# pierre-borie/Benlsip.jl

Hardware: AMD Instinct MI355X
Metric: PCG subproblems/sec + achieved HBM GB/s, dense m=65536 n=4096 fp64 (higher is better)
Workload: dtype f64

## Files before the change

benlsip.jl_amd/csrc/bh_api.hip:

```cpp
#include "../../include/benlsip_hip.h"
#include "bh_cauchy_plan.h"
#include "bh_free_image_plan.h"
#include "bh_gram_ingest_plan.h"
#include "bh_kernels.hip.h"
#include "bh_launch_ahead.h"
#include "bh_pcg_plan.h"

#include <dlfcn.h>
#include <fcntl.h>
#include <rccl/rccl.h>
#include <sched.h>
#include <sys/mman.h>
#include <unistd.h>

#include <algorithm>
#include <atomic>
#include <chrono>
#include <cmath>
#include <cstdio>
#include <cstdlib>
#include <cstring>
#include <array>
#include <initializer_list>
#include <string>
#include <thread>
#include <tuple>
#include <vector>

using namespace bh;

static uint64_t g_kernel_launches = 0;
static uint64_t g_mask_epoch = 0;
#undef hipLaunchKernelGGL
#define hipLaunchKernelGGL(kernelName, ...) do { ++g_kernel_launches; hipLaunchKernelGGLInternal((kernelName), __VA_ARGS__); } while (0)

namespace {

struct CgWorkspace {
    int64_t n_pad = 0;
    double *w = nullptr, *r = nullptr, *v = nullptr, *p = nullptr, *Hp = nullptr, *g = nullptr, *wl = nullptr, *wu = nullptr;
    double *x = nullptr, *s = nullptr, *xlow = nullptr, *xupp = nullptr;
    double* hw = nullptr;
    double *p2 = nullptr, *gpart = nullptr, *rvpart = nullptr;
    double *r2 = nullptr, *hpx = nullptr, *hpx_tail = nullptr;
    double* slab = nullptr;
    double* scalars = nullptr;
    CgState* d_state = nullptr;
    volatile unsigned long long* h_mirror = nullptr;
    unsigned long long* d_mirror = nullptr;
    unsigned tag = 0;
    unsigned long long* d_reroute = nullptr;
    unsigned long long reroute_seq = 0;
    double* d_trace = nullptr;
    int64_t trace_cap = 0;
};

struct PeerShm {
    std::atomic<int> arrive;
    std::atomic<int> generation;
    int failed;
    hipIpcMemHandle_t handle[kMaxPeers];
};
struct PeerComm {
    bool active = false;
    bool broken = false;
    void* inbox = nullptr;
    size_t inbox_bytes = 0;
    void* peer_base[kMaxPeers] = {};
    volatile unsigned long long* h_err = nullptr;
    PeerShm* shm = nullptr;
    PeerArgs args{};
};
constexpr int64_t kPeerCap = 1 << 16;
constexpr int kPeerBlkCap = (int)(kPeerCap / (2 * kPeerBlockChunks));
constexpr size_t kPeerSlotBytes = (size_t)2 * kMaxPeers * kPeerCap * sizeof(double);
constexpr size_t kPeerFlagBytes = (size_t)2 * kMaxPeers * kPeerBlkCap * sizeof(unsigned long long);
constexpr size_t kPeerScalBytes = kPeerFlagBytes;

struct AsyncUpload {
    std::thread worker;
    int32_t rc = BH_OK;
    std::string detail;
    hipStream_t s_copy = nullptr, s_xpose = nullptr;
    double* staging[2] = {nullptr, nullptr};
    hipEvent_t copied[2] = {nullptr, nullptr}, freed[2] = {nullptr, nullptr};
// ... 9 lines not shown
};

struct Ctx {
    bool init = false;
    int device = -1;
    int flags = 0;
    int n_cu = 0;
    hipStream_t own_stream = nullptr;
    hipStream_t stream = nullptr;
    std::string detail;
    int64_t opt_blocks_per_cu = 0;
    int64_t opt_batch = 0;
    int64_t opt_chol_downdate = 0;
    int64_t opt_cauchy_image = 1;
    int64_t opt_cauchy_image_max_ma = 64;
    int64_t opt_cauchy_image_refresh = 0;
    int64_t opt_cauchy_fused = 1;
    int64_t opt_cauchy_gram_eq = 0;
    int64_t opt_cauchy_gram = 0;
    int64_t opt_linv_refine = 1;
    int64_t opt_cauchy_gemm = 1;
    int64_t opt_gram_cg_fused = 0;
    int64_t opt_gram_mfma = 1;
    int64_t opt_ls_from_cg = 1;
    int64_t opt_step_from_cg = 0;
    struct { const void* H = nullptr; const double* w = nullptr; const double* gm = nullptr; } hw_note;
    struct { const void* H = nullptr; const double* s = nullptr; const double* g = nullptr; const double* gm = nullptr; } gm_note;
    int64_t opt_fold_init = 1;
    int64_t opt_final_sync = 0;
    int64_t opt_host_copy_kernels = 1;
    int64_t opt_cg_fused = 1;
    int64_t opt_proj_form = 1;
    int64_t opt_upload_chunk_mb = 64;
    int64_t opt_free_image = 1;
    int64_t opt_gram_ingest = 0;
    int64_t opt_ev_stride = 8;
    void* rccl_lib = nullptr;
    ncclComm_t comm = nullptr;
    int rank = 0, nranks = 1;
    ncclResult_t (*p_ncclGetUniqueId)(ncclUniqueId*) = nullptr;
    ncclResult_t (*p_ncclCommInitRank)(ncclComm_t*, int, ncclUniqueId, int) = nullptr;
    ncclResult_t (*p_ncclCommDestroy)(ncclComm_t) = nullptr;
    ncclResult_t (*p_ncclAllReduce)(const void*, void*, size_t, ncclDataType_t, ncclRedOp_t, ncclComm_t, hipStream_t) = nullptr;
    const char* (*p_ncclGetErrorString)(ncclResult_t) = nullptr;
    PeerComm peer;
    int comm_path = 0;
    CgWorkspace cg;
    double* scratch_dev = nullptr;
    struct PooledImage { double* ptr; int64_t doubles; };
    std::vector<PooledImage> image_pool;
    int64_t opt_image_pool = 2;
    int64_t image_pool_hits = 0;
    AsyncUpload* upload_cache = nullptr;
    int64_t h2d_bytes = 0, d2h_bytes = 0, h2d_calls = 0, d2h_calls = 0;
    volatile unsigned long long* mbox_h = nullptr;
    unsigned long long* mbox_d = nullptr;
    unsigned long long mbox_seq = 0;
    double* rbuf = nullptr;
    int64_t rbuf_cap = 0;
    int live_hess = 0;
    bool reform_vlds_attr_set = false;
    bool vlds_attr_set = false;
    bool cgp_vlds_attr_set = false;
    bool trsm_lds_granted = false;
    size_t trsv_lds_granted = 0;
};
// ... 273 lines not shown

namespace {

int32_t ensure_cg_workspace(int64_t n_pad, int64_t trace_cap) {
    CgWorkspace& c = g_ctx.cg;
    if (c.n_pad < n_pad) {
        double** vecs[] = {&c.w, &c.r, &c.v, &c.p, &c.Hp, &c.s, &c.x, &c.xlow, &c.xupp, &c.g, &c.wl, &c.wu, &c.hw, &c.p2, &c.gpart, &c.rvpart,
                           &c.r2, &c.hpx, &c.hpx_tail};
        constexpr int NV = 19;
        dev_free(c.slab);
        c.slab = nullptr;
        g_ctx.hw_note = {};
        BH_TRY(dev_alloc(&c.slab, NV * n_pad + 8));
        BH_HIP(hipMemsetAsync(c.slab, 0, (size_t)(NV * n_pad + 8) * sizeof(double), g_ctx.stream));
        for (int i = 0; i < NV; ++i) *vecs[i] = c.slab + (int64_t)i * n_pad;
        c.scalars = c.slab + NV * n_pad;
        c.n_pad = n_pad;
    }
    if (!c.d_state) {
        BH_TRY(dev_alloc(&c.d_state, 1));
        BH_HIP(hipMemsetAsync(c.d_state, 0, sizeof(CgState), g_ctx.stream));
        void* hp = nullptr;
        BH_HIP(hipHostMalloc(&hp, 64, hipHostMallocMapped | hipHostMallocCoherent));
        memset(hp, 0, 64);
        c.h_mirror = reinterpret_cast<volatile unsigned long long*>(hp);
        void* dp = nullptr;
        BH_HIP(hipHostGetDevicePointer(&dp, hp, 0));
        c.d_mirror = reinterpret_cast<unsigned long long*>(dp);
    }
    if (!c.d_reroute) {
        BH_TRY(dev_alloc(&c.d_reroute, 1));
        BH_HIP(hipMemsetAsync(c.d_reroute, 0, sizeof(unsigned long long), g_ctx.stream));
    }
    if (trace_cap > c.trace_cap) {
        dev_free(c.d_trace);
        c.d_trace = nullptr;
        BH_TRY(dev_alloc(&c.d_trace, 4 * trace_cap));
        c.trace_cap = trace_cap;
    }
    return BH_OK;
}

int32_t check_peer_error();
int32_t hess_ready(bh_hess* H);

int32_t wait_mirror(CgWorkspace& c, unsigned tag, int target, MirrorWord* out, int iter_target = 0) {
    const auto t0 = std::chrono::steady_clock::now();
    unsigned long long spins = 0;
    auto reached = [&](unsigned long long w, MirrorWord* m) {
        if (((w >> 48) & 0xffffu) != (tag & 0xffffu)) return false;
        m->status = (int)((w >> 44) & 0xf);
        m->done = (int)((w >> 40) & 0xf);
        m->iter = (int)((w >> 20) & 0xfffff);
        m->n_hmul = (int)(w & 0xfffff);
        return m->done != 0 || m->n_hmul >= target || (iter_target > 0 && m->iter >= iter_target);
    };
    while (true) {
        if (reached(*c.h_mirror, out)) return BH_OK;
        __builtin_ia32_pause();
        if ((++spins & 0xffff) == 0) {
            if (g_ctx.peer.active && *g_ctx.peer.h_err != 0ull) return check_peer_error();
            hipError_t q = hipStreamQuery(g_ctx.stream);
            if (q != hipSuccess && q != hipErrorNotReady) return fail(BH_ERR_HIP, std::string("CG loop: ") + hipGetErrorString(q));
            if (q == hipSuccess) {
                MirrorWord m2{};
                if (!reached(*c.h_mirror, &m2)) return fail(BH_ERR_HIP, "internal: stream drained but the loop state did not reach the launch target");
// ... 756 lines not shown
        default: return "unknown error code";
    }
}

const char* bh_last_error_detail(void) { return g_ctx.detail.c_str(); }

int32_t bh_init(int32_t device, int32_t flags) {
    if (g_ctx.init) {
        if (device != g_ctx.device)
            return fail(BH_ERR_INVALID_ARG, "bh_init: already initialised on another device (bh_shutdown first)");
        g_ctx.flags = flags;
        return BH_OK;
    }
    int count = 0;
    hipError_t e = hipGetDeviceCount(&count);
    if (e != hipSuccess || count <= 0) return fail(BH_ERR_NO_DEVICE, "hipGetDeviceCount found no device");
    if (device < 0 || device >= count) return fail(BH_ERR_INVALID_ARG, "device ordinal out of range");
    BH_HIP(hipSetDevice(device));
    hipDeviceProp_t prop;
    BH_HIP(hipGetDeviceProperties(&prop, device));
    g_ctx.n_cu = prop.multiProcessorCount;
    g_ctx.device = device;
    g_ctx.flags = flags;
    BH_HIP(hipStreamCreateWithFlags(&g_ctx.own_stream, hipStreamNonBlocking));
    g_ctx.stream = g_ctx.own_stream;
    BH_TRY(dev_alloc(&g_ctx.scratch_dev, 1024));
    BH_TRY(mbox_ensure());
    if (const char* s = getenv("BH_HOST_COPY_KERNELS")) g_ctx.opt_host_copy_kernels = atoll(s) ? 1 : 0;
    if (const char* s = getenv("BH_BLOCKS_PER_CU")) g_ctx.opt_blocks_per_cu = std::min<int64_t>(std::max<int64_t>(0, atoll(s)), kMaxBlocksPerCu);
    if (const char* s = getenv("BH_PCG_BATCH")) g_ctx.opt_batch = std::max<int64_t>(0, atoll(s));
    if (const char* s = getenv("BH_PROJ_FORM")) g_ctx.opt_proj_form = atoll(s) ? 1 : 0;
    if (const char* s = getenv("BH_CG_FUSED")) g_ctx.opt_cg_fused = std::min<int64_t>(std::max<int64_t>(0, atoll(s)), 2);
    if (const char* s = getenv("BH_FINAL_SYNC")) g_ctx.opt_final_sync = atoll(s) ? 1 : 0;
    if (const char* s = getenv("BH_FREE_IMAGE")) g_ctx.opt_free_image = std::min<int64_t>(std::max<int64_t>(0, atoll(s)), 2);
    g_ctx.init = true;
    return BH_OK;
}

static void peer_release(bool with_barrier);

int32_t bh_shutdown(void) {
    if (!g_ctx.init) return BH_OK;
    (void)hipStreamSynchronize(g_ctx.stream);
    if (g_ctx.comm && g_ctx.p_ncclCommDestroy) { g_ctx.p_ncclCommDestroy(g_ctx.comm); g_ctx.comm = nullptr; }
    if (g_ctx.peer.active) peer_release(true);
    g_ctx.comm_path = 0;
    CgWorkspace& c = g_ctx.cg;
    dev_free(c.slab); dev_free(c.d_state); dev_free(c.d_trace); dev_free(c.d_reroute);
    if (c.h_mirror) (void)hipHostFree(const_cast<unsigned long long*>(c.h_mirror));
    c = CgWorkspace();
    dev_free(g_ctx.scratch_dev); g_ctx.scratch_dev = nullptr;
    dev_free(g_ctx.rbuf); g_ctx.rbuf = nullptr; g_ctx.rbuf_cap = 0;
    if (g_ctx.mbox_h) { (void)hipHostFree(const_cast<unsigned long long*>(g_ctx.mbox_h)); g_ctx.mbox_h = nullptr; g_ctx.mbox_d = nullptr; }
    async_upload_destroy(g_ctx.upload_cache); g_ctx.upload_cache = nullptr;
    for (auto& im : g_ctx.image_pool) dev_free(im.ptr);
    g_ctx.image_pool.clear();
    if (g_ctx.own_stream) (void)hipStreamDestroy(g_ctx.own_stream);
    g_ctx.own_stream = nullptr; g_ctx.stream = nullptr;
    if (g_pin.base) { (void)hipHostFree(g_pin.base); g_pin = PinArena(); }
    g_ctx.vlds_attr_set = false; g_ctx.cgp_vlds_attr_set = false; g_ctx.reform_vlds_attr_set = false; g_ctx.trsm_lds_granted = false; g_ctx.trsv_lds_granted = 0;
    g_ctx.init = false; g_ctx.rank = 0; g_ctx.nranks = 1;
    return BH_OK;
}

int32_t bh_set_stream(void* hip_stream) {
    BH_REQUIRE_INIT();
    BH_TRY(sync_flush());
    g_ctx.stream = hip_stream ? reinterpret_cast<hipStream_t>(hip_stream) : g_ctx.own_stream;
    return BH_OK;
}

int32_t bh_synchronize(void) {
    BH_REQUIRE_INIT();
    BH_TRY(sync_flush());
    return BH_OK;
}

int32_t bh_device_info(char* name_out, int64_t name_cap, int32_t* n_cu, char* arch_out, int64_t arch_cap) {
    BH_REQUIRE_INIT();
    hipDeviceProp_t prop;
    BH_HIP(hipGetDeviceProperties(&prop, g_ctx.device));
    if (name_out && name_cap > 0) { strncpy(name_out, prop.name, (size_t)name_cap - 1); name_out[name_cap - 1] = 0; }
    if (arch_out && arch_cap > 0) { strncpy(arch_out, prop.gcnArchName, (size_t)arch_cap - 1); arch_out[arch_cap - 1] = 0; }
    if (n_cu) *n_cu = prop.multiProcessorCount;
    return BH_OK;
}

int32_t bh_set_option(const char* key, int64_t value) {
    if (!key) return fail(BH_ERR_INVALID_ARG, "NULL key");
    if (!strcmp(key, "blocks_per_cu")) {
        if (value < 0 || value > kMaxBlocksPerCu) return fail(BH_ERR_INVALID_ARG, "blocks_per_cu must be 0 (default) .. 8");
        g_ctx.opt_blocks_per_cu = value;
        return BH_OK;
    }
    if (!strcmp(key, "pcg_batch")) { g_ctx.opt_batch = std::max<int64_t>(0, value); return BH_OK; }
    if (!strcmp(key, "proj_form")) { g_ctx.opt_proj_form = value ? 1 : 0; return BH_OK; }
    if (!strcmp(key, "fold_init")) { g_ctx.opt_fold_init = value ? 1 : 0; return BH_OK; }
    if (!strcmp(key, "cg_fused")) {
        if (value < 0 || value > 2) return fail(BH_ERR_INVALID_ARG, "cg_fused is 0, 1 (box constraints) or 2 (also linear equalities)");
        g_ctx.opt_cg_fused = value;
        return BH_OK;
    }
    if (!strcmp(key, "final_sync")) { g_ctx.opt_final_sync = value ? 1 : 0; return BH_OK; }
    if (!strcmp(key, "host_copy_kernels")) { g_ctx.opt_host_copy_kernels = value ? 1 : 0; return BH_OK; }
    if (!strcmp(key, "ls_from_cg")) { g_ctx.opt_ls_from_cg = value ? 1 : 0; return BH_OK; }
    if (!strcmp(key, "step_from_cg")) { g_ctx.opt_step_from_cg = value ? 1 : 0; return BH_OK; }
    if (!strcmp(key, "gram_mfma")) { g_ctx.opt_gram_mfma = value; return BH_OK; }
    if (!strcmp(key, "chol_downdate")) { g_ctx.opt_chol_downdate = value ? 1 : 0; return BH_OK; }
    if (!strcmp(key, "cauchy_image")) { g_ctx.opt_cauchy_image = value ? 1 : 0; return BH_OK; }
    if (!strcmp(key, "cauchy_gram")) { g_ctx.opt_cauchy_gram = value ? 1 : 0; return BH_OK; }
    if (!strcmp(key, "cauchy_gram_eq")) {
        if (value != 0 && value != 1) return fail(BH_ERR_INVALID_ARG, "cauchy_gram_eq is 0 or 1");
        g_ctx.opt_cauchy_gram_eq = value;
        return BH_OK;
    }
    if (!strcmp(key, "gram_cg_fused")) {
        if (value != 0) BH_REQUIRE_INIT();
        if (value != 0 && value != 1) return fail(BH_ERR_INVALID_ARG, "gram_cg_fused is 0 or 1");
        g_ctx.opt_gram_cg_fused = value;
        return BH_OK;
    }
    if (!strcmp(key, "cauchy_image_refresh")) {
        if (value < 0) return fail(BH_ERR_INVALID_ARG, "cauchy_image_refresh is 0 (never) or the number of passes between two re-formations");
        g_ctx.opt_cauchy_image_refresh = value;
        return BH_OK;
    }
    if (!strcmp(key, "cauchy_fused")) { g_ctx.opt_cauchy_fused = value ? 1 : 0; return BH_OK; }
    if (!strcmp(key, "linv_refine")) { g_ctx.opt_linv_refine = value ? 1 : 0; return BH_OK; }
    if (!strcmp(key, "cauchy_gemm")) { g_ctx.opt_cauchy_gemm = value ? 1 : 0; return BH_OK; }
    if (!strcmp(key, "cauchy_image_max_ma")) { g_ctx.opt_cauchy_image_max_ma = std::min<int64_t>(std::max<int64_t>(0, value), 64); return BH_OK; }
    if (!strcmp(key, "image_pool")) {
        if (value < 0 || value > 8) return fail(BH_ERR_INVALID_ARG, "image_pool must be 0..8");
        g_ctx.opt_image_pool = value;
        while ((int64_t)g_ctx.image_pool.size() > value) { dev_free(g_ctx.image_pool.back().ptr); g_ctx.image_pool.pop_back(); }
        return BH_OK;
// ... 986 lines not shown
        cold = 1;
    }
    p.sched.first = launch_ahead_first(H->last_n_hmul, cold);
    return p;
}

static void pcg_use_free_image(PcgRun& r) {
    bh_hess* H = r.H; CgWorkspace& c = r.c;
    const FreeImageBook& b = H->fi;
    r.fi_use = true;
    r.og = c.x; r.owl = c.xlow; r.owu = c.xupp; r.ow = c.s;
    r.ofix = nullptr;
    r.on = (int)b.nfree; r.onch = (int)(round_up(b.nfree, 16) / 2);
    r.old = b.ldf;
    pcg_fused_geometry(r.plan, H, r.onch, r.on);
    H->call_bytes = free_image_bytes(H);
    c.reroute_seq += 1;
}

static int32_t pcg_fused_stream(PcgRun& r, int j) {
    bh_hess* H = r.H; CgWorkspace& c = r.c; const PcgPlan& p = r.plan;
    RowStreamArgs ra = rs_args(H, p.nrows, nullptr);
    ra.partials = H->partials;
    if (p.gram) { ra.J = H->G; ra.d_rows = p.nrows; ra.mu = 1.0; ra.partials = nullptr; ra.t_out = c.Hp; }
    if (r.fi_use) { ra.J = H->Jf; ra.ld = r.old; ra.nchunks = r.onch; }
    if (p.sel.fuse_gen) { ra.v = c.p; ra.negate = 0; }
    else { ra.v = r.og; ra.negate = 1; ra.negmask = r.ofix; }
    CgFuse& f = ra.cf;
    f.st = c.d_state; f.j = j; f.n = r.on; f.max_iter = p.max_iter; f.init_done = p.sel.gen_linv ? 2 : p.sel.fuse_gen ? 1 : 0; f.vv_off = p.vv_off;
    f.vvec = c.v; f.p_old = p.pbuf[(j - 1) & 1]; f.p_new = p.pbuf[j & 1];
    f.rvpart = p.rvbuf[(j - 1) & 1]; f.nrv = p.nrv;
    f.w = r.ow; f.wl = r.owl; f.wu = r.owu;
    if (r.fi_use) { f.reroute = c.d_reroute; f.reroute_seq = c.reroute_seq; }
    f.sqpart = H->sq_partials; f.gpart = H->sq_partials + H->g_cap;
    f.kappa2 = r.a.kappa2; f.atol_f2b = r.a.atol_f2b;
    f.trace = r.a.trace; f.trace_cap = r.a.trace_cap; f.mirror = r.a.mirror; f.tag = r.a.tag;
    int slot = -1;
    const bool expect_stop = j == r.expect_stop_at || j > p.max_iter || (r.expect_stop_at == 0 && j > 1);
    BH_TRY(profile_begin(H, j - 1, &slot));
    if (p.gram) launch_gram_cg(p.cfg, ra, p.grid, r.s, expect_stop);
    else launch_row_stream_cgp(p.cfg, ra, p.grid, r.s, expect_stop);
    if (slot >= 0) BH_HIP(hipEventRecord(H->ev[2 * slot + 1], r.s));
    return BH_OK;
}

static int32_t pcg_fused_update(PcgRun& r, int j) {
    bh_hess* H = r.H; bh_proj* P = r.P; CgWorkspace& c = r.c; const PcgPlan& p = r.plan; hipStream_t s = r.s;
    const int nblk = p.nblk, grid = p.grid;
    CgUpdArgs u{};
    u.st = c.d_state; u.j = j; u.partials = H->partials; u.ld = r.old; u.nchunks = r.onch; u.G = grid; u.Gs = grid; u.Gq = grid;
    u.sqpart = H->sq_partials; u.gpart = H->sq_partials + H->g_cap; u.rvpart_in = p.rvbuf[(j - 1) & 1]; u.rvpart_out = p.rvbuf[j & 1]; u.nrv = p.nrv;
    u.p = p.pbuf[j & 1]; u.w = r.ow; u.hw = r.hw; u.r = c.r; u.g = r.og; u.v = c.v; u.fixrank = r.ofix;
    if (r.fi_use) { u.map = H->fi_map; u.w_full = r.wp; u.reroute = c.d_reroute; u.reroute_seq = c.reroute_seq; }
    u.n = r.on; u.atol_neg = r.a.atol_neg; u.trace = r.a.trace; u.trace_cap = r.a.trace_cap; u.mirror = r.a.mirror; u.tag = r.a.tag;
    if (p.gram) { u.partials = c.Hp; u.Gs = 1; }
    if (!p.sel.fuse_gen) {
        if (p.sel.peer_fused) hipLaunchKernelGGL((cg_reduce_update_kernel<false, true>), dim3(nblk), dim3(256), 0, s, u, g_ctx.peer.args);
        else hipLaunchKernelGGL((cg_reduce_update_kernel<false, false>), dim3(nblk), dim3(256), 0, s, u, PeerArgs{});
        return BH_OK;
    }
    if (p.sel.rccl_gen) {
        const int n_pad = r.a.n_pad;
        hipLaunchKernelGGL(reduce_partials_sq_kernel, dim3(nblk), dim3(256), 0, s, (const double*)H->partials, H->ld, H->nchunks, grid,
                           c.hpx, (const double*)H->sq_partials, n_pad, (const CgState*)c.d_state, j);
        BH_HIP(hipGetLastError());
        BH_TRY(allreduce_inplace(c.hpx, (int64_t)n_pad + 2, H));
        u.partials = c.hpx; u.Gs = 1; u.sqpart = c.hpx + n_pad; u.Gq = 1;
    }
    u.A = P->Ad; u.ldA = P->ldA; u.mA = (int)P->mA; u.tpart = P->tpart; u.init_in_memory = p.sel.gen_linv ? 0 : 1;
    if (p.sel.peer_fused) hipLaunchKernelGGL((cg_reduce_update_kernel<true, true>), dim3(nblk), dim3(256), 0, s, u, g_ctx.peer.args);
    else hipLaunchKernelGGL((cg_reduce_update_kernel<true, false>), dim3(nblk), dim3(256), 0, s, u, PeerArgs{});
    ProjArgs pa = proj_args(P, c.d_state, true);
    pa.tpart = P->tpart; pa.tpart_nblk = nblk; pa.rvpart = p.rvbuf[j & 1]; pa.fused_j = j;
    if (p.sel.gen_linv) {
        pa.W = P->W; pa.nch_pad = H->nchunks; pa.Mgram = p.sel.linv_refine ? P->M : nullptr;
        hipLaunchKernelGGL((proj_apply_linv_kernel<false>), dim3((unsigned)p.nrv), dim3(256), 0, s, pa, (const double*)c.r, c.v);
        return BH_OK;
    }
    hipLaunchKernelGGL(trsv_small_kernel, dim3(1), dim3(256), 0, s, pa);
    hipLaunchKernelGGL((proj_left_mul_tr_kernel<true, 4>), dim3((p.nch_v + 63) / 64), dim3(256), 0, s, pa, (const double*)c.r, c.v);
    return BH_OK;
}

static int32_t pcg_fused_first(PcgRun& r) {
    bh_hess* H = r.H; bh_proj* P = r.P; CgWorkspace& c = r.c; const PcgPlan& p = r.plan; hipStream_t s = r.s;
    if (r.fi_use) {
        FreeGatherArgs ga{};
        ga.g = r.a.g; ga.wl = r.a.wl; ga.wu = r.a.wu; ga.fixrank = P->fixrank; ga.map = H->fi_map;
        ga.gc = c.x; ga.wlc = c.xlow; ga.wuc = c.xupp; ga.wc = c.s; ga.w = r.wp;
        ga.n = r.a.n; ga.n_pad = r.a.n_pad; ga.nfree = r.on;
        ga.reroute = c.d_reroute; ga.seq = c.reroute_seq; ga.mirror = r.a.mirror; ga.tag = r.a.tag;
        hipLaunchKernelGGL(free_image_gather_kernel, dim3((unsigned)((r.a.n_pad + 255) / 256)), dim3(256), 0, s, ga);
    }
    if (p.sel.gen_linv) {
        if (!P->linv_valid) {
            hipLaunchKernelGGL(tri_inv_small_kernel, dim3(1), dim3(256), 0, s, (const double*)P->Lr, (int)P->mA, P->W);
            P->linv_valid = true;
        }
        ProjArgs pa = proj_args(P, nullptr, true);
        hipLaunchKernelGGL(proj_left_mul_kernel, dim3((unsigned)P->mA), dim3(256), 0, s, pa, r.a.g);
        pa.tpart = P->tw; pa.tpart_nblk = 1; pa.rvpart = p.rvbuf[0]; pa.vvpart = p.rvbuf[0] + p.vv_off; pa.p_out = c.p;
        pa.W = P->W; pa.nch_pad = H->nchunks; pa.Mgram = p.sel.linv_refine ? P->M : nullptr; pa.fused_j = 0;
        hipLaunchKernelGGL((proj_apply_linv_kernel<true>), dim3((unsigned)p.nrv), dim3(256), 0, s, pa, r.a.g, c.v);
    } else if (p.sel.fuse_gen) {
        hipLaunchKernelGGL((cg_init_kernel<false>), dim3(1), dim3(CG_T), 0, s, r.a);
        BH_TRY(launch_project(P, c.r, c.v, c.d_state));
        hipLaunchKernelGGL(cg_init_finish_kernel, dim3(1), dim3(CG_T), 0, s, r.a);
    }
    return pcg_fused_stream(r, 1);
}

static int32_t pcg_fused_unit(PcgRun& r, int index) {
    BH_TRY(pcg_fused_update(r, index + 1));
    BH_TRY(pcg_fused_stream(r, index + 2));
    BH_HIP(hipGetLastError());
    return BH_OK;
}

static int32_t pcg_rccl_box_stream(PcgRun& r, int j) {
    bh_hess* H = r.H; CgWorkspace& c = r.c; const PcgPlan& p = r.plan; const CgArgs& a = r.a;
    RowStreamArgs ra = rs_args(H, p.nrows, nullptr);
    ra.partials = H->partials;
    ra.v = a.g; ra.negate = 1; ra.negmask = a.fixrank;
    CgFuse& f = ra.cf;
    f.st = c.d_state; f.j = j; f.n = a.n; f.max_iter = p.max_iter; f.init_done = 0;
    f.p_old = p.pbuf[(j - 1) & 1]; f.p_new = p.pbuf[j & 1];
// ... 1165 lines not shown
```

benlsip.jl_amd/csrc/bh_cg.hip.h:

```cpp
#pragma once
#include <hip/hip_runtime.h>
#include <stdint.h>
#include "bh_reduce.hip.h"

namespace bh {

constexpr int CG_T = 1024;

struct CgArgs {
    CgState* st;
    double* w; double* r; double* v; double* p;
    const double* Hp;
    const double* g;
    const double* wl; const double* wu;
    const int* fixrank;
    int n;
    int n_pad;
    int w_in_ws;
    int max_iter;
    double kappa2, atol_neg, atol_f2b;
    double* trace; int trace_cap;
    double* hw;
    unsigned long long* mirror;
    unsigned tag;
};

__device__ __forceinline__ double f2b_term(double p, double w, double wl, double wu, double atol) {
    double g = __longlong_as_double(0x7ff0000000000000ll);
    if (p <= -atol) g = __ddiv_rn(__dsub_rn(wl, w), p);
    else if (p >= atol) g = __ddiv_rn(__dsub_rn(wu, w), p);
    return g;
}

__device__ __forceinline__ int cg_final_status(const CgState* st) {
    if (st->approx_solved) return 0;
    if (st->outside_region) return 1;
    if (st->neg_curvature) return 2;
    if (st->iter == st->max_iter) return 3;
    return 4;
}

__device__ __forceinline__ void publish_state(const CgArgs& a, const CgState* st) {
    if (a.mirror == nullptr) return;
    const unsigned long long wv = ((unsigned long long)(a.tag & 0xffffu) << 48) | ((unsigned long long)(st->status & 0xf) << 44) |
                                  ((unsigned long long)(st->done & 0xf) << 40) | ((unsigned long long)(st->iter & 0xfffff) << 20) |
                                  (unsigned long long)(st->n_hmul & 0xfffff);
    if (st->done) {
        const unsigned long long tw = ((unsigned long long)(st->margin_kind & 0xf) << 48) | ((unsigned long long)(st->tie_flags & 0xff) << 40) |
                                      ((unsigned long long)(st->tie_first & 0xfffff) << 20) | (unsigned long long)(st->margin_at & 0xfffff);
        __hip_atomic_store(a.mirror + 1, tw, __ATOMIC_RELAXED, __HIP_MEMORY_SCOPE_SYSTEM);
        __hip_atomic_store(a.mirror + 2, (unsigned long long)__double_as_longlong(st->min_margin), __ATOMIC_RELAXED, __HIP_MEMORY_SCOPE_SYSTEM);
    }
    __hip_atomic_store(a.mirror, wv, __ATOMIC_RELAXED, __HIP_MEMORY_SCOPE_SYSTEM);
}

__device__ __forceinline__ void publish_word(unsigned long long* mirror, unsigned tag, int status, int done, int iter, int n_hmul,
                                             const TieRegs& tr) {
    if (mirror == nullptr) return;
    const unsigned long long wv = ((unsigned long long)(tag & 0xffffu) << 48) | ((unsigned long long)(status & 0xf) << 44) |
                                  ((unsigned long long)(done & 0xf) << 40) | ((unsigned long long)(iter & 0xfffff) << 20) |
                                  (unsigned long long)(n_hmul & 0xfffff);
    if (done) {
        const unsigned long long tw = ((unsigned long long)(tr.margin_kind & 0xf) << 48) | ((unsigned long long)(tr.tie_flags & 0xff) << 40) |
                                      ((unsigned long long)(tr.tie_first & 0xfffff) << 20) | (unsigned long long)(tr.margin_at & 0xfffff);
        __hip_atomic_store(mirror + 1, tw, __ATOMIC_RELAXED, __HIP_MEMORY_SCOPE_SYSTEM);
        __hip_atomic_store(mirror + 2, (unsigned long long)__double_as_longlong(tr.min_margin), __ATOMIC_RELAXED, __HIP_MEMORY_SCOPE_SYSTEM);
    }
    __hip_atomic_store(mirror, wv, __ATOMIC_RELAXED, __HIP_MEMORY_SCOPE_SYSTEM);
}
__device__ __forceinline__ int cg_status_of(int approx_solved, int outside_region, int neg_curvature, int iter, int max_iter) {
    if (approx_solved) return 0;
    if (outside_region) return 1;
    if (neg_curvature) return 2;
// ... 471 lines not shown
```

benlsip.jl_amd/csrc/bh_cgfuse.hip.h:

```cpp
#pragma once
#include <hip/hip_runtime.h>
#include <stdint.h>
#include "bh_reduce.hip.h"
#include "bh_cg.hip.h"
#include "bh_comm.hip.h"

namespace bh {

struct CgUpdArgs {
    CgState* st;
    int j;
    const double* partials; int64_t ld; int nchunks; int G;
    int Gs, Gq;
    const double* sqpart;
    const double* gpart;
    const double* rvpart_in;
    double* rvpart_out;
    int nrv;
    const double* p;
    double* w; double* hw;
    double* r; const double* g;
    double* v;
    const int* fixrank;
    int n;
    double atol_neg;
    double* trace; int trace_cap;
    unsigned long long* mirror; unsigned tag;
    const double* A; int64_t ldA; int mA;
    double* tpart;
    int init_in_memory;
    const int* map; double* w_full;
    const unsigned long long* reroute; unsigned long long reroute_seq;
};

template <bool GEN, bool PEER>
__global__ __launch_bounds__(256) void cg_reduce_update_kernel(CgUpdArgs a, PeerArgs pa) {
    CgState* st = a.st;
    if (st->stop_at != 0 && a.j > st->stop_at) return;
    if (a.reroute != nullptr && *a.reroute == a.reroute_seq) return;
    __shared__ double2 sm[16][17];
    __shared__ double rvs[16];
    __shared__ double2 rsm[16];
    const int tid = threadIdx.x, cl = tid & 15, rl = tid >> 4;
    const int c = blockIdx.x * 16 + cl;
    const bool valid = c < a.nchunks;
    const int64_t ld2 = a.ld >> 1;
    const double QNAN = __longlong_as_double(0x7ff8000000000000ll);

    const bool upd = (rl == 0) && valid;
    const bool from_g = (a.j == 1 && !a.init_in_memory);
    double2 pk = make_double2(0.0, 0.0), wk = pk, hwk = pk, rk = pk;
    int2 fr = make_int2(-1, -1);
    if (upd) {
        pk = reinterpret_cast<const double2*>(a.p)[c];
        if (from_g) {
            rk = reinterpret_cast<const double2*>(a.g)[c];
        } else {
            rk = reinterpret_cast<const double2*>(a.r)[c];
            wk = reinterpret_cast<const double2*>(a.w)[c];
            if (a.hw != nullptr) hwk = reinterpret_cast<const double2*>(a.hw)[c];
        }
    }
    TieRegs tr;
    tr.load(st);
    const int max_iter = st->max_iter;
    const double rtv_state = st->rtv;
    LaneBatch<8> b_sq, b_gp, b_rv;
    b_sq.issue(a.sqpart, a.Gq);
    b_gp.issue(a.gpart, a.G);
    b_rv.issue(a.rvpart_in, a.nrv);
    const double2* P2 = reinterpret_cast<const double2*>(a.partials);
    const int cc = min(c, a.nchunks - 1);
    SlabBatch sb;
    sb.issue(P2, ld2, cc, rl, a.Gs);
    double2 arow[4];
    if (GEN) {
        const double2* A2 = reinterpret_cast<const double2*>(a.A);
        const int64_t ldA2 = a.ldA >> 1;
#pragma unroll
        for (int k = 0; k < 4; ++k) arow[k] = A2[(int64_t)min(rl + 16 * k, a.mA - 1) * ldA2 + cc];
    }
    int2 mp = make_int2(-1, -1);
    if (!GEN && upd && a.map != nullptr) mp = reinterpret_cast<const int2*>(a.map)[c];
    if (upd && a.fixrank != nullptr) fr = reinterpret_cast<const int2*>(a.fixrank)[c];

    const double2 acc = sb.fold(P2, ld2, cc, rl, a.Gs);
    sm[rl][cl] = acc;

    double pHp = wave_sum(b_sq.fold_sum(a.sqpart, a.Gq));
    if (PEER) {
        __shared__ int s_timeout;
        __shared__ double2 xs[kMaxPeers][16];
        __shared__ double ps[kMaxPeers];
        if (tid == 0) s_timeout = 0;
        __syncthreads();
        if (rl == 0) {
            double2 t = sm[0][cl];
#pragma unroll
            for (int q = 1; q < 16; ++q) { t.x += sm[q][cl].x; t.y += sm[q][cl].y; }
// ... 112 lines not shown
    } else {
        __syncthreads();
        if (cont) {
            const double2 rm = rsm[cl];
#pragma unroll
            for (int k = 0; k < 4; ++k) {
                const int i = rl + 16 * k;
                if (i < a.mA) {
                    double prod = valid ? fma(arow[k].y, rm.y, arow[k].x * rm.x) : 0.0;
                    prod = row16_sum(prod);
                    if (cl == 0) a.tpart[(int64_t)blockIdx.x * a.mA + i] = prod;
                }
            }
        }
    }

    if (blockIdx.x == 0 && tid == 0) {
        st->pHp = pHp; st->gamma = gamma; st->alpha = alpha; st->n_hmul = a.j; st->rtv = rtv;
        st->neg_curvature = neg; st->outside_region = outside; st->need_proj = 0; st->iter = a.j;
        tr.note_step_a(pHp, a.atol_neg, alpha, gamma, a.j);
        tr.store(st);
        if (a.trace != nullptr && a.j <= a.trace_cap) {
            double* row = a.trace + 4 * (int64_t)(a.j - 1);
            row[0] = pHp; row[1] = alpha; row[2] = (neg && !add_w) ? QNAN : gamma; row[3] = rtv;
        }
        int status = 4;
        if (!cont) {
            status = cg_status_of(0, outside, neg, a.j, max_iter);
            st->approx_solved = 0; st->done = 1; st->stop_at = a.j;
            st->status = status;
        }
        publish_word(a.mirror, a.tag, status, cont ? 0 : 1, a.j, a.j, tr);
    }
}

}
```

benlsip.jl_amd/csrc/bh_freeimg.hip.h:

```cpp
#pragma once
#include <hip/hip_runtime.h>
#include <stdint.h>
#include "bh_reduce.hip.h"

namespace bh {

__global__ __launch_bounds__(256) void free_image_build_kernel(const double* __restrict__ J, int64_t ld, int64_t nrows,
                                                               const int* __restrict__ map, double* __restrict__ Jf, int64_t ldf) {
    const int nch = (int)(ldf >> 1);
    for (int64_t row = blockIdx.x; row < nrows; row += gridDim.x) {
        const double* __restrict__ src = J + row * ld;
        double2* __restrict__ dst = reinterpret_cast<double2*>(Jf + row * ldf);
        for (int c = threadIdx.x; c < nch; c += 256) {
            const int2 m = reinterpret_cast<const int2*>(map)[c];
            double2 x = make_double2(0.0, 0.0);
            if (m.x >= 0 && m.y == m.x + 1 && (m.x & 1) == 0) {
                const dvec2 t = __builtin_nontemporal_load(reinterpret_cast<const dvec2*>(src + m.x));
                x = make_double2(t.x, t.y);
            } else {
                if (m.x >= 0) x.x = __builtin_nontemporal_load(src + m.x);
                if (m.y >= 0) x.y = __builtin_nontemporal_load(src + m.y);
            }
            dst[c] = x;
        }
    }
}

__global__ __launch_bounds__(256) void free_image_move_kernel(double* __restrict__ Jf, int64_t ldf, int64_t nrows, int nfree_new, int k,
                                                              const int* __restrict__ dst_of_tail, int* __restrict__ map) {
    const int64_t total = nrows * (int64_t)k;
    for (int64_t idx = (int64_t)blockIdx.x * 256 + threadIdx.x; idx < total; idx += (int64_t)gridDim.x * 256) {
        const int64_t row = idx / k;
        const int t = (int)(idx - row * k);
        const int dst = dst_of_tail[t];
        double* __restrict__ rp = Jf + row * ldf;
        const double x = rp[nfree_new + t];
        if (dst >= 0) rp[dst] = x;
        rp[nfree_new + t] = 0.0;
    }
    if (blockIdx.x == 0) {
        for (int t = threadIdx.x; t < k; t += 256) {
            const int dst = dst_of_tail[t];
            const int var = map[nfree_new + t];
            if (dst >= 0) map[dst] = var;
            map[nfree_new + t] = -1;
        }
    }
}

constexpr int kCgReroute = 15;
struct FreeGatherArgs {
    const double* g; const double* wl; const double* wu;
    const int* fixrank;
    const int* map;
    double* gc; double* wlc; double* wuc;
    double* wc;
    double* w;
    int n, n_pad, nfree;
    unsigned long long* reroute; unsigned long long seq;
    unsigned long long* mirror; unsigned tag;
};

__global__ __launch_bounds__(256) void free_image_gather_kernel(FreeGatherArgs a) {
    const int i = blockIdx.x * 256 + threadIdx.x;
    if (i < a.n_pad) {
        const int m = (i < a.nfree) ? a.map[i] : -1;
        a.gc[i] = (m >= 0) ? a.g[m] : 0.0;
        a.wlc[i] = (m >= 0) ? a.wl[m] : 0.0;
        a.wuc[i] = (m >= 0) ? a.wu[m] : 0.0;
        a.wc[i] = 0.0;
    }
    if (i < a.n && a.fixrank[i] >= 0) {
        a.w[i] = 0.0;
        const double gi = a.g[i];
        if (!(fabs(gi) <= 1.7976931348623157e308)) {
            *a.reroute = a.seq;
            if (a.mirror != nullptr) {
                const unsigned long long wv = ((unsigned long long)(a.tag & 0xffffu) << 48) | ((unsigned long long)kCgReroute << 44) | (1ull << 40);
                __hip_atomic_store(a.mirror, wv, __ATOMIC_RELAXED, __HIP_MEMORY_SCOPE_SYSTEM);
            }
        }
    }
}

}
```

benlsip.jl_amd/csrc/bh_matvec.hip.h:

```cpp
#pragma once
#include <hip/hip_runtime.h>
#include <stdint.h>
#include "bh_reduce.hip.h"
#include "bh_cg.hip.h"

namespace bh {

enum { MODE_JV = 0, MODE_JTV = 1, MODE_FUSED = 2 };

struct CgFuse {
    CgState* st;
    int j;
    int init_done;
    int vv_off;
    int n, max_iter;
    const double* vvec;
    const double* p_old;
    double* p_new;
    const double* rvpart;
    int nrv;
    const double* w;
    const double* wl; const double* wu;
    double* sqpart;
    double* gpart;
    double kappa2, atol_f2b;
    double* trace; int trace_cap;
    unsigned long long* mirror; unsigned tag;
    const double* gpart_in;
    const double* Hp;
    int sq_index;
    const double* r_old;
    double* r_new;
    double* w_rw;
    double* hw;
    const double* g;
    const int* fixrank;
    double atol_neg;
    const unsigned long long* reroute; unsigned long long reroute_seq;
};

struct RowStreamArgs {
    const double* J;
    int64_t ld;
    int64_t nrows;
    int64_t d_rows;
    int nchunks;
    const double* v;
    const double* u;
    double* t_out;
    double* partials;
    double* sq_partials;
    double mu;
    const CgState* state;
    int accumulate;
    int weighted_u;
    int negate;
    const int* negmask;
    CgFuse cf;
};

template <int T, int CPT, int R, int MODE, int NT = 1, int PF = 1, int VL = 0, int CGP = 0>
__global__ __launch_bounds__(T) void row_stream_kernel(RowStreamArgs a) {
    static_assert(NT == 1 && PF == 1, "plain loads (NT = 0) and the single register buffer (PF = 0) lost their A/Bs and were removed");
    if (!CGP && a.state != nullptr && a.state->done) return;
    if (CGP && a.cf.j > 1 && a.cf.st->stop_at != 0 && a.cf.j > a.cf.st->stop_at + (CGP == 3 ? 1 : 0)) return;
    if ((CGP == 1 || CGP == 2) && a.cf.reroute != nullptr && *a.cf.reroute == a.cf.reroute_seq) return;
    constexpr int NW = T / 64;
    __shared__ double red[2][R][NW];
    __shared__ double pro[2][NW];
    extern __shared__ __attribute__((aligned(16))) double2 v_lds[];

    const int tid = threadIdx.x, lane = tid & 63, wave = tid >> 6;
    const int64_t ld2 = a.ld >> 1;
    const double2* __restrict__ J2 = reinterpret_cast<const double2*>(a.J);
    const int64_t ngroups = (a.nrows + R - 1) / R;
    const int64_t G = gridDim.x;

    bool act[CPT];
    double2 vv[CPT], zz[CPT];
#pragma unroll
    for (int k = 0; k < CPT; ++k) act[k] = (tid + k * T) < a.nchunks;

    double2 A[R][CPT], B[R][CPT];
    double sq_acc = 0.0;
    int buf = 0;

    auto load_group = [&](double2 (&dst)[R][CPT], int64_t grp) {
#pragma unroll
        for (int r = 0; r < R; ++r) {
            const int64_t row = grp * R + r;
            const bool rv = row < a.nrows;
            const double2* rp = J2 + (rv ? row : 0) * ld2;
#pragma unroll
            for (int k = 0; k < CPT; ++k) {
                dst[r][k] = make_double2(0.0, 0.0);
                if (rv && act[k]) {
                    const dvec2 t = __builtin_nontemporal_load(reinterpret_cast<const dvec2*>(rp + tid + k * T));
                    dst[r][k] = make_double2(t.x, t.y);
                }
// ... 40 lines not shown
            if (tid < R && row < a.nrows) a.t_out[row] = a.accumulate ? a.t_out[row] + mine : mine;
        }
#pragma unroll
        for (int r = 0; r < R; ++r) {
            const int64_t row = grp * R + r;
            const bool rv = row < a.nrows;
            if (MODE == MODE_JV) {
                if (rv) {
                    const double wgt = (row < a.d_rows) ? 1.0 : a.mu;
                    sq_acc = fma(wgt * s[r], s[r], sq_acc);
                }
            } else {
                double coef;
                if (MODE == MODE_JTV) coef = rv ? (a.weighted_u && row >= a.d_rows ? a.mu * a.u[row] : a.u[row]) : 0.0;
                else {
                    coef = (row < a.d_rows) ? s[r] : a.mu * s[r];
                    if (CGP && rv) sq_acc = fma(coef, s[r], sq_acc);
                }
#pragma unroll
                for (int k = 0; k < CPT; ++k) {
                    zz[k].x = fma(coef, X[r][k].x, zz[k].x);
                    zz[k].y = fma(coef, X[r][k].y, zz[k].y);
                }
            }
        }
    };

    int64_t g = blockIdx.x;
#pragma unroll
    for (int k = 0; k < CPT; ++k) {
        vv[k] = make_double2(0.0, 0.0);
        zz[k] = make_double2(0.0, 0.0);
    }
    if (!CGP || a.cf.j == 1) {
        if (g < ngroups) load_group(A, g);
        int2 nm[CPT];
#pragma unroll
        for (int k = 0; k < CPT; ++k) {
            const int c = tid + k * T;
            nm[k] = make_int2(-1, -1);
            if (MODE != MODE_JTV && act[k]) {
                vv[k] = reinterpret_cast<const double2*>(a.v)[c];
                if (a.negate && a.negmask != nullptr) nm[k] = reinterpret_cast<const int2*>(a.negmask)[c];
            }
        }
        if (MODE != MODE_JTV && a.negate) {
#pragma unroll
            for (int k = 0; k < CPT; ++k) {
                vv[k].x = (nm[k].x >= 0) ? 0.0 : -vv[k].x;
                vv[k].y = (nm[k].y >= 0) ? 0.0 : -vv[k].y;
            }
        }
    }
    if (CGP == 3) {
        const CgFuse& f = a.cf;
        CgState* st = f.st;
        const double QNAN = __longlong_as_double(0x7ff8000000000000ll);
        OpMinNan opmin;
        double2 wnew[CPT];
        bool own[CPT];
#pragma unroll
        for (int k = 0; k < CPT; ++k) {
            const int c = tid + k * T;
            own[k] = act[k] && ((c / CPT) % (int)G) == (int)blockIdx.x;
            wnew[k] = make_double2(0.0, 0.0);
        }
        if (f.j == 1) {
            double rtv0 = 0.0;
#pragma unroll
            for (int k = 0; k < CPT; ++k) { rtv0 = fma(vv[k].x, vv[k].x, rtv0); rtv0 = fma(vv[k].y, vv[k].y, rtv0); }
            rtv0 = wave_sum(rtv0);
            if (lane == 0) pro[0][wave] = rtv0;
            __syncthreads();
            double t = 0.0;
            for (int w2 = 0; w2 < NW; ++w2) t += pro[0][w2];
#pragma unroll
            for (int k = 0; k < CPT; ++k) {
                if (!own[k]) continue;
                const int c = tid + k * T;
                double2 gk = reinterpret_cast<const double2*>(f.g)[c];
                if (2 * c >= f.n) gk.x = 0.0;
                if (2 * c + 1 >= f.n) gk.y = 0.0;
                reinterpret_cast<double2*>(f.r_new)[c] = gk;
                reinterpret_cast<double2*>(f.w_rw)[c] = make_double2(0.0, 0.0);
// ... 181 lines not shown
                }
            }
            const double rtv = st->rtv, tol_cg = st->tol_cg;
            TieRegs tr;
            tr.load(st);
            const int outside_prev = st->outside_region, neg_prev = st->neg_curvature;
            const double rtv_next = wave_fixed_sum(f.rvpart, f.nrv);
            const bool solved = fabs(rtv_next) < tol_cg;
            const bool stop = solved || f.j > f.max_iter;
            const double beta = __ddiv_rn(rtv_next, rtv);
            if (blockIdx.x == 0 && tid == 0) {
                tr.note(TIE_TOL, rel_margin(fabs(rtv_next), tol_cg), f.j - 1);
                tr.store(st);
                if (f.trace != nullptr && f.j - 1 <= f.trace_cap) f.trace[4 * (int64_t)(f.j - 2) + 3] = rtv_next;
                st->iter = f.j;
                int status = 4;
                if (stop) {
                    status = cg_status_of(solved ? 1 : 0, outside_prev, neg_prev, f.j, f.max_iter);
                    st->beta = beta; st->rtv = rtv_next; st->approx_solved = solved ? 1 : 0;
                    st->done = 1; st->stop_at = f.j - 1;
                    st->status = status;
                }
                publish_word(f.mirror, f.tag, status, stop ? 1 : 0, f.j, f.j - 1, tr);
            }
            if (stop) return;
            if (CGP == 2 && g < ngroups) load_group(A, g);
#pragma unroll
            for (int k = 0; k < CPT; ++k) {
                vv[k].x = __dadd_rn(-vk[k].x, __dmul_rn(beta, po[k].x));
                vv[k].y = __dadd_rn(-vk[k].y, __dmul_rn(beta, po[k].y));
            }
        }
        OpMinNan opmin;
        double gm = __longlong_as_double(0x7ff0000000000000ll);
#pragma unroll
        for (int k = 0; k < CPT; ++k) {
            const int c = tid + k * T;
            if (!act[k] || ((c / CPT) % (int)G) != (int)blockIdx.x) continue;
            reinterpret_cast<double2*>(f.p_new)[c] = vv[k];
            double2 wk = make_double2(0.0, 0.0);
            if (f.j > 1) wk = reinterpret_cast<const double2*>(f.w)[c];
            const double2 lo = reinterpret_cast<const double2*>(f.wl)[c], hi = reinterpret_cast<const double2*>(f.wu)[c];
            if (2 * c < f.n) gm = opmin(gm, f2b_term(vv[k].x, wk.x, lo.x, hi.x, f.atol_f2b));
            if (2 * c + 1 < f.n) gm = opmin(gm, f2b_term(vv[k].y, wk.y, lo.y, hi.y, f.atol_f2b));
        }
        gm = wave_min(gm);
        if (NW > 1) {
            if (lane == 0) pro[1][wave] = gm;
            __syncthreads();
            gm = pro[1][0];
            for (int w2 = 1; w2 < NW; ++w2) gm = opmin(gm, pro[1][w2]);
        }
        if (tid == 0) f.gpart[blockIdx.x] = gm;
    }
    if (VL && MODE != MODE_JTV) {
#pragma unroll
        for (int k = 0; k < CPT; ++k) v_lds[k * T + tid] = vv[k];
    }

    if (g < ngroups) {
        while (true) {
            int64_t gn = g + G;
            if (gn < ngroups) load_group(B, gn);
            process(A, g);
            if (gn >= ngroups) break;
            g = gn;
            gn = g + G;
            if (gn < ngroups) load_group(A, gn);
            process(B, g);
            if (gn >= ngroups) break;
            g = gn;
        }
    }

// ... 146 lines not shown
```

Baseline: 1789.

## Fold free-image gather into first CG matvec and add last-block stop verdict

```diff
diff --git a/benlsip.jl_amd/csrc/bh_api.hip b/benlsip.jl_amd/csrc/bh_api.hip
--- a/benlsip.jl_amd/csrc/bh_api.hip
+++ b/benlsip.jl_amd/csrc/bh_api.hip
@@ -51,6 +51,7 @@
     unsigned tag = 0;
     unsigned long long* d_reroute = nullptr;
     unsigned long long reroute_seq = 0;
+    unsigned* d_ticket = nullptr;
     double* d_trace = nullptr;
     int64_t trace_cap = 0;
 };
@@ -126,6 +127,7 @@
     int64_t opt_cg_fused = 1;
     int64_t opt_proj_form = 1;
     int64_t opt_upload_chunk_mb = 64;
+    int64_t opt_cg_verdict = 1;
     int64_t opt_free_image = 1;
     int64_t opt_gram_ingest = 0;
     int64_t opt_ev_stride = 8;
@@ -465,6 +467,10 @@
         BH_TRY(dev_alloc(&c.d_reroute, 1));
         BH_HIP(hipMemsetAsync(c.d_reroute, 0, sizeof(unsigned long long), g_ctx.stream));
     }
+    if (!c.d_ticket) {
+        BH_TRY(dev_alloc(&c.d_ticket, 1));
+        BH_HIP(hipMemsetAsync(c.d_ticket, 0, sizeof(unsigned), g_ctx.stream));
+    }
     if (trace_cap > c.trace_cap) {
         dev_free(c.d_trace);
         c.d_trace = nullptr;
@@ -1287,6 +1293,7 @@
     if (const char* s = getenv("BH_PROJ_FORM")) g_ctx.opt_proj_form = atoll(s) ? 1 : 0;
     if (const char* s = getenv("BH_CG_FUSED")) g_ctx.opt_cg_fused = std::min<int64_t>(std::max<int64_t>(0, atoll(s)), 2);
     if (const char* s = getenv("BH_FINAL_SYNC")) g_ctx.opt_final_sync = atoll(s) ? 1 : 0;
+    if (const char* s = getenv("BH_CG_VERDICT")) g_ctx.opt_cg_verdict = atoll(s) ? 1 : 0;
     if (const char* s = getenv("BH_FREE_IMAGE")) g_ctx.opt_free_image = std::min<int64_t>(std::max<int64_t>(0, atoll(s)), 2);
     g_ctx.init = true;
     return BH_OK;
@@ -1301,7 +1308,7 @@
     if (g_ctx.peer.active) peer_release(true);
     g_ctx.comm_path = 0;
     CgWorkspace& c = g_ctx.cg;
-    dev_free(c.slab); dev_free(c.d_state); dev_free(c.d_trace); dev_free(c.d_reroute);
+    dev_free(c.slab); dev_free(c.d_state); dev_free(c.d_trace); dev_free(c.d_reroute); dev_free(c.d_ticket);
     if (c.h_mirror) (void)hipHostFree(const_cast<unsigned long long*>(c.h_mirror));
     c = CgWorkspace();
     dev_free(g_ctx.scratch_dev); g_ctx.scratch_dev = nullptr;
@@ -1356,6 +1363,7 @@
         g_ctx.opt_cg_fused = value;
         return BH_OK;
     }
+    if (!strcmp(key, "cg_verdict")) { g_ctx.opt_cg_verdict = value ? 1 : 0; return BH_OK; }
     if (!strcmp(key, "final_sync")) { g_ctx.opt_final_sync = value ? 1 : 0; return BH_OK; }
     if (!strcmp(key, "host_copy_kernels")) { g_ctx.opt_host_copy_kernels = value ? 1 : 0; return BH_OK; }
     if (!strcmp(key, "ls_from_cg")) { g_ctx.opt_ls_from_cg = value ? 1 : 0; return BH_OK; }
@@ -2408,6 +2416,11 @@
     f.rvpart = p.rvbuf[(j - 1) & 1]; f.nrv = p.nrv;
     f.w = r.ow; f.wl = r.owl; f.wu = r.owu;
     if (r.fi_use) { f.reroute = c.d_reroute; f.reroute_seq = c.reroute_seq; }
+    if (r.fi_use && j == 1) {
+        f.gmap = H->fi_map; f.g_full = r.a.g; f.wl_full = r.a.wl; f.wu_full = r.a.wu;
+        f.gc = c.x; f.wlc = c.xlow; f.wuc = c.xupp;
+        f.fixrank_full = r.P->fixrank; f.w_full = r.wp; f.n_full = r.a.n;
+    }
     f.sqpart = H->sq_partials; f.gpart = H->sq_partials + H->g_cap;
     f.kappa2 = r.a.kappa2; f.atol_f2b = r.a.atol_f2b;
     f.trace = r.a.trace; f.trace_cap = r.a.trace_cap; f.mirror = r.a.mirror; f.tag = r.a.tag;
@@ -2430,6 +2443,9 @@
     if (r.fi_use) { u.map = H->fi_map; u.w_full = r.wp; u.reroute = c.d_reroute; u.reroute_seq = c.reroute_seq; }
     u.n = r.on; u.atol_neg = r.a.atol_neg; u.trace = r.a.trace; u.trace_cap = r.a.trace_cap; u.mirror = r.a.mirror; u.tag = r.a.tag;
     if (p.gram) { u.partials = c.Hp; u.Gs = 1; }
+    const int js = j + 1;
+    const bool expect_stop = js == r.expect_stop_at || js > p.max_iter || r.expect_stop_at == 0;
+    if (g_ctx.opt_cg_verdict && expect_stop && !p.gram && !p.sel.fuse_gen && !p.sel.peer_fused) { u.verdict = 1; u.ticket = c.d_ticket; }
     if (!p.sel.fuse_gen) {
         if (p.sel.peer_fused) hipLaunchKernelGGL((cg_reduce_update_kernel<false, true>), dim3(nblk), dim3(256), 0, s, u, g_ctx.peer.args);
         else hipLaunchKernelGGL((cg_reduce_update_kernel<false, false>), dim3(nblk), dim3(256), 0, s, u, PeerArgs{});
@@ -2460,14 +2476,6 @@
 
 static int32_t pcg_fused_first(PcgRun& r) {
     bh_hess* H = r.H; bh_proj* P = r.P; CgWorkspace& c = r.c; const PcgPlan& p = r.plan; hipStream_t s = r.s;
-    if (r.fi_use) {
-        FreeGatherArgs ga{};
-        ga.g = r.a.g; ga.wl = r.a.wl; ga.wu = r.a.wu; ga.fixrank = P->fixrank; ga.map = H->fi_map;
-        ga.gc = c.x; ga.wlc = c.xlow; ga.wuc = c.xupp; ga.wc = c.s; ga.w = r.wp;
-        ga.n = r.a.n; ga.n_pad = r.a.n_pad; ga.nfree = r.on;
-        ga.reroute = c.d_reroute; ga.seq = c.reroute_seq; ga.mirror = r.a.mirror; ga.tag = r.a.tag;
-        hipLaunchKernelGGL(free_image_gather_kernel, dim3((unsigned)((r.a.n_pad + 255) / 256)), dim3(256), 0, s, ga);
-    }
     if (p.sel.gen_linv) {
         if (!P->linv_valid) {
             hipLaunchKernelGGL(tri_inv_small_kernel, dim3(1), dim3(256), 0, s, (const double*)P->Lr, (int)P->mA, P->W);
diff --git a/benlsip.jl_amd/csrc/bh_cg.hip.h b/benlsip.jl_amd/csrc/bh_cg.hip.h
--- a/benlsip.jl_amd/csrc/bh_cg.hip.h
+++ b/benlsip.jl_amd/csrc/bh_cg.hip.h
@@ -39,6 +39,8 @@
     if (st->iter == st->max_iter) return 3;
     return 4;
 }
+
+constexpr int kCgReroute = 15;
 
 __device__ __forceinline__ void publish_state(const CgArgs& a, const CgState* st) {
     if (a.mirror == nullptr) return;
diff --git a/benlsip.jl_amd/csrc/bh_cgfuse.hip.h b/benlsip.jl_amd/csrc/bh_cgfuse.hip.h
--- a/benlsip.jl_amd/csrc/bh_cgfuse.hip.h
+++ b/benlsip.jl_amd/csrc/bh_cgfuse.hip.h
@@ -31,6 +31,7 @@
     int init_in_memory;
     const int* map; double* w_full;
     const unsigned long long* reroute; unsigned long long reroute_seq;
+    int verdict; unsigned* ticket;
 };
 
 template <bool GEN, bool PEER>
@@ -65,6 +66,10 @@
     tr.load(st);
     const int max_iter = st->max_iter;
     const double rtv_state = st->rtv;
+    const bool verdict = !GEN && !PEER && a.verdict != 0;
+    double tol_cg = 0.0;
+    if (verdict) tol_cg = st->tol_cg;
+    const TieRegs tr_in = tr;
     LaneBatch<8> b_sq, b_gp, b_rv;
     b_sq.issue(a.sqpart, a.Gq);
     b_gp.issue(a.gpart, a.G);
@@ -243,6 +248,46 @@
         }
         publish_word(a.mirror, a.tag, status, cont ? 0 : 1, a.j, a.j, tr);
     }
+
+    if (!GEN && !PEER) {
+        if (verdict && cont && tid < 64) {
+            unsigned last = 0;
+            if (tid == 0) {
+                __builtin_amdgcn_fence(__ATOMIC_RELEASE, "agent");
+                asm volatile("s_waitcnt vmcnt(0)" ::: "memory");
+                const unsigned t = __hip_atomic_fetch_add(a.ticket, 1u, __ATOMIC_RELAXED, __HIP_MEMORY_SCOPE_AGENT);
+                last = (t + 1u == gridDim.x) ? 1u : 0u;
+            }
+            last = (unsigned)__builtin_amdgcn_readfirstlane((int)last);
+            if (last) {
+                __builtin_amdgcn_fence(__ATOMIC_ACQUIRE, "agent");
+                asm volatile("s_waitcnt vmcnt(0)" ::: "memory");
+                const int lane = tid;
+                double acc = 0.0;
+                for (int i = lane; i < (int)gridDim.x; i += 64)
+                    acc += __hip_atomic_load(a.rvpart_out + i, __ATOMIC_RELAXED, __HIP_MEMORY_SCOPE_AGENT);
+                const double rtv_next = wave_sum(acc);
+                const bool solved = fabs(rtv_next) < tol_cg;
+                const bool stop = solved || a.j + 1 > max_iter;
+                if (tid == 0) {
+                    __hip_atomic_store(a.ticket, 0u, __ATOMIC_RELAXED, __HIP_MEMORY_SCOPE_AGENT);
+                    if (stop) {
+                        TieRegs tv = tr_in;
+                        tv.note_step_a(pHp, a.atol_neg, alpha, gamma, a.j);
+                        tv.note(TIE_TOL, rel_margin(fabs(rtv_next), tol_cg), a.j);
+                        tv.store(st);
+                        if (a.trace != nullptr && a.j <= a.trace_cap) a.trace[4 * (int64_t)(a.j - 1) + 3] = rtv_next;
+                        const int status = cg_status_of(solved ? 1 : 0, 0, 0, a.j + 1, max_iter);
+                        st->iter = a.j + 1;
+                        st->beta = __ddiv_rn(rtv_next, rtv); st->rtv = rtv_next; st->approx_solved = solved ? 1 : 0;
+                        st->done = 1; st->stop_at = a.j;
+                        st->status = status;
+                        publish_word(a.mirror, a.tag, status, 1, a.j + 1, a.j, tv);
+                    }
+                }
+            }
+        }
+    }
 }
 
 }
diff --git a/benlsip.jl_amd/csrc/bh_freeimg.hip.h b/benlsip.jl_amd/csrc/bh_freeimg.hip.h
--- a/benlsip.jl_amd/csrc/bh_freeimg.hip.h
+++ b/benlsip.jl_amd/csrc/bh_freeimg.hip.h
@@ -48,39 +48,5 @@
     }
 }
 
-constexpr int kCgReroute = 15;
-struct FreeGatherArgs {
-    const double* g; const double* wl; const double* wu;
-    const int* fixrank;
-    const int* map;
-    double* gc; double* wlc; double* wuc;
-    double* wc;
-    double* w;
-    int n, n_pad, nfree;
-    unsigned long long* reroute; unsigned long long seq;
-    unsigned long long* mirror; unsigned tag;
-};
-
-__global__ __launch_bounds__(256) void free_image_gather_kernel(FreeGatherArgs a) {
-    const int i = blockIdx.x * 256 + threadIdx.x;
-    if (i < a.n_pad) {
-        const int m = (i < a.nfree) ? a.map[i] : -1;
-        a.gc[i] = (m >= 0) ? a.g[m] : 0.0;
-        a.wlc[i] = (m >= 0) ? a.wl[m] : 0.0;
-        a.wuc[i] = (m >= 0) ? a.wu[m] : 0.0;
-        a.wc[i] = 0.0;
-    }
-    if (i < a.n && a.fixrank[i] >= 0) {
-        a.w[i] = 0.0;
-        const double gi = a.g[i];
-        if (!(fabs(gi) <= 1.7976931348623157e308)) {
-            *a.reroute = a.seq;
-            if (a.mirror != nullptr) {
-                const unsigned long long wv = ((unsigned long long)(a.tag & 0xffffu) << 48) | ((unsigned long long)kCgReroute << 44) | (1ull << 40);
-                __hip_atomic_store(a.mirror, wv, __ATOMIC_RELAXED, __HIP_MEMORY_SCOPE_SYSTEM);
-            }
-        }
-    }
-}
 
 }
diff --git a/benlsip.jl_amd/csrc/bh_matvec.hip.h b/benlsip.jl_amd/csrc/bh_matvec.hip.h
--- a/benlsip.jl_amd/csrc/bh_matvec.hip.h
+++ b/benlsip.jl_amd/csrc/bh_matvec.hip.h
@@ -36,7 +36,11 @@
     const double* g;
     const int* fixrank;
     double atol_neg;
-    const unsigned long long* reroute; unsigned long long reroute_seq;
+    unsigned long long* reroute; unsigned long long reroute_seq;
+    const int* gmap;
+    const double* g_full; const double* wl_full; const double* wu_full;
+    double* gc; double* wlc; double* wuc;
+    const int* fixrank_full; double* w_full; int n_full;
 };
 
 struct RowStreamArgs {
@@ -64,7 +68,7 @@
     static_assert(NT == 1 && PF == 1, "plain loads (NT = 0) and the single register buffer (PF = 0) lost their A/Bs and were removed");
     if (!CGP && a.state != nullptr && a.state->done) return;
     if (CGP && a.cf.j > 1 && a.cf.st->stop_at != 0 && a.cf.j > a.cf.st->stop_at + (CGP == 3 ? 1 : 0)) return;
-    if ((CGP == 1 || CGP == 2) && a.cf.reroute != nullptr && *a.cf.reroute == a.cf.reroute_seq) return;
+    if ((CGP == 1 || CGP == 2) && a.cf.j > 1 && a.cf.reroute != nullptr && *a.cf.reroute == a.cf.reroute_seq) return;
     constexpr int NW = T / 64;
     __shared__ double red[2][R][NW];
     __shared__ double pro[2][NW];
@@ -171,8 +175,75 @@
         vv[k] = make_double2(0.0, 0.0);
         zz[k] = make_double2(0.0, 0.0);
     }
+    double gm_first = __longlong_as_double(0x7ff0000000000000ll);
     if (!CGP || a.cf.j == 1) {
+        const bool fold_gather = (CGP == 1 || CGP == 2) && a.cf.gmap != nullptr;
+        int fr0 = -1;
+        int2 gm[CPT];
+        if (fold_gather) {
+            const int64_t i0 = (int64_t)blockIdx.x * T + tid;
+            if (i0 < a.cf.n_full) fr0 = a.cf.fixrank_full[i0];
+#pragma unroll
+            for (int k = 0; k < CPT; ++k) {
+                gm[k] = make_int2(-1, -1);
+                if (act[k]) gm[k] = reinterpret_cast<const int2*>(a.cf.gmap)[tid + k * T];
+            }
+        }
         if (g < ngroups) load_group(A, g);
+        if (fold_gather) {
+            const CgFuse& f = a.cf;
+            const int64_t i0 = (int64_t)blockIdx.x * T + tid;
+#pragma unroll
+            for (int k = 0; k < CPT; ++k) {
+                const int c = tid + k * T;
+                if (2 * c >= f.n) gm[k].x = -1;
+                if (2 * c + 1 >= f.n) gm[k].y = -1;
+                vv[k] = make_double2(f.g_full[max(gm[k].x, 0)], f.g_full[max(gm[k].y, 0)]);
+            }
+            const double g0 = f.g_full[fr0 >= 0 ? i0 : 0];
+            OpMinNan opmin1;
+#pragma unroll
+            for (int k = 0; k < CPT; ++k) {
+                const int c = tid + k * T;
+                const bool own = act[k] && ((c / CPT) % (int)G) == (int)blockIdx.x;
+                double2 lo = make_double2(0.0, 0.0), hi = lo;
+                if (own) {
+                    const int mx = max(gm[k].x, 0), my = max(gm[k].y, 0);
+                    lo = make_double2(f.wl_full[mx], f.wl_full[my]);
+                    hi = make_double2(f.wu_full[mx], f.wu_full[my]);
+                }
+                if (gm[k].x < 0) { vv[k].x = 0.0; lo.x = 0.0; hi.x = 0.0; }
+                if (gm[k].y < 0) { vv[k].y = 0.0; lo.y = 0.0; hi.y = 0.0; }
+                if (own) {
+                    reinterpret_cast<double2*>(f.gc)[c] = vv[k];
+                    reinterpret_cast<double2*>(f.wlc)[c] = lo;
+                    reinterpret_cast<double2*>(f.wuc)[c] = hi;
+                }
+                vv[k].x = -vv[k].x; vv[k].y = -vv[k].y;
+                if (own) {
+                    if (2 * c < f.n) gm_first = opmin1(gm_first, f2b_term(vv[k].x, 0.0, lo.x, hi.x, f.atol_f2b));
+                    if (2 * c + 1 < f.n) gm_first = opmin1(gm_first, f2b_term(vv[k].y, 0.0, lo.y, hi.y, f.atol_f2b));
+                }
+            }
+            bool hand_back = false;
+            if (fr0 >= 0) {
+                f.w_full[i0] = 0.0;
+                hand_back = !(fabs(g0) <= 1.7976931348623157e308);
+            }
+            for (int64_t i = i0 + G * T; i < f.n_full; i += G * T) {
+                if (f.fixrank_full[i] >= 0) {
+                    f.w_full[i] = 0.0;
+                    if (!(fabs(f.g_full[i]) <= 1.7976931348623157e308)) hand_back = true;
+                }
+            }
+            if (hand_back) {
+                *f.reroute = f.reroute_seq;
+                if (f.mirror != nullptr) {
+                    const unsigned long long wv = ((unsigned long long)(f.tag & 0xffffu) << 48) | ((unsigned long long)kCgReroute << 44) | (1ull << 40);
+                    __hip_atomic_store(f.mirror, wv, __ATOMIC_RELAXED, __HIP_MEMORY_SCOPE_SYSTEM);
+                }
+            }
+        } else {
         int2 nm[CPT];
 #pragma unroll
         for (int k = 0; k < CPT; ++k) {
@@ -189,6 +260,7 @@
                 vv[k].x = (nm[k].x >= 0) ? 0.0 : -vv[k].x;
                 vv[k].y = (nm[k].y >= 0) ? 0.0 : -vv[k].y;
             }
+        }
         }
     }
     if (CGP == 3) {
@@ -436,7 +508,7 @@
             }
         }
         OpMinNan opmin;
-        double gm = __longlong_as_double(0x7ff0000000000000ll);
+        double gm = gm_first;
 #pragma unroll
         for (int k = 0; k < CPT; ++k) {
             const int c = tid + k * T;
@@ -444,6 +516,7 @@
             reinterpret_cast<double2*>(f.p_new)[c] = vv[k];
             double2 wk = make_double2(0.0, 0.0);
             if (f.j > 1) wk = reinterpret_cast<const double2*>(f.w)[c];
+            if (f.j == 1 && f.gmap != nullptr) continue;
             const double2 lo = reinterpret_cast<const double2*>(f.wl)[c], hi = reinterpret_cast<const double2*>(f.wu)[c];
             if (2 * c < f.n) gm = opmin(gm, f2b_term(vv[k].x, wk.x, lo.x, hi.x, f.atol_f2b));
             if (2 * c + 1 < f.n) gm = opmin(gm, f2b_term(vv[k].y, wk.y, lo.y, hi.y, f.atol_f2b));
```

Result: no change. 1789 (-0.0%).
